# fugue-project/fugue

Measured on AMD Instinct MI355X. Metric: rows_per_sec_transform_fuguesql_groupby_join, higher is better.
Workload: dtype int64+fp64; 1 GPU; model=fuguesql[transform+groupby(sum,count)+join+filter], global_rows=125000000, rows_per_gpu=125000000, n_groups=1000000, dim_rows=1000000, parallelism=dp1, out_rows=1000000

## Files before the change

fugue_amd/hip/csrc/bindings.cpp:

```cpp
#include <torch/extension.h>

#include <c10/hip/HIPStream.h>
#include <hip/hip_runtime.h>

#include <cstdlib>
#include <cstdio>
#include <cstring>
#include <limits>
#include <vector>

#include "relational.h"

namespace {

hipStream_t current_stream() {
  return (hipStream_t)c10::hip::getCurrentHIPStream().stream();
}

void check_gpu(const at::Tensor& t, const char* name) {
  TORCH_CHECK(t.is_cuda(), name, " must be on the GPU");
  TORCH_CHECK(t.is_contiguous(), name, " must be contiguous");
}

const bool* opt_valid_ptr(const c10::optional<at::Tensor>& v) {
// ... 621 lines not shown
  }
  TORCH_CHECK((bin_group_base.slice(0, 1) - bin_group_base.slice(0, 0, nbins))
                      .max()
                      .item<int64_t>() <= 65536,
              "a bin wider than 65536 ids does not fit 16-bit ids");
  auto stream = current_stream();
  auto counts = at::empty({ntiles, nbins}, pos.options());
  launch_scatter_bin_count(pos.data_ptr<int32_t>(), n, (int)tile,
                           bin_offsets.data_ptr<int64_t>(), (int)nbins,
                           counts.data_ptr<int32_t>(), stream);
  auto row_incl = counts.cumsum(1, at::kLong);
  auto start = row_incl - counts;
  auto tile_delta = (bin_offsets.slice(0, 0, nbins).unsqueeze(0) +
                     (counts.cumsum(0, at::kLong) - counts) - start)
                        .to(at::kInt)
                        .contiguous();
  auto tile_start = at::cat({start, row_incl.slice(1, nbins - 1, nbins)}, 1)
                        .to(at::kShort)
                        .contiguous();
  launch_scatter_tile_prep_compact(
      pos.data_ptr<int32_t>(), n, (int)tile, bin_offsets.data_ptr<int64_t>(),
      bin_group_base.data_ptr<int64_t>(), (int)nbins,
      tile_delta.data_ptr<int32_t>(), gid.data_ptr<int32_t>(),
      (uint16_t*)rank.data_ptr<int16_t>(), (uint16_t*)rel.data_ptr<int16_t>(),
      keep_gid ? gid_new.data_ptr<int32_t>() : nullptr, stream);
  std::vector<at::Tensor> res = {rank, rel, tile_start, tile_delta};
  if (keep_gid) res.push_back(gid_new);
  return res;
}

at::Tensor scatter_tile_compact(at::Tensor vals, at::Tensor rank,
                                at::Tensor tile_start, at::Tensor tile_delta,
                                int64_t tile, int64_t threads,
                                c10::optional<at::Tensor> out_opt) {
  if (out_opt.has_value()) {
    check_gpu(*out_opt, "out");
    TORCH_CHECK(out_opt->scalar_type() == at::kDouble &&
                    out_opt->is_contiguous() &&
                    out_opt->numel() == rank.numel(),
                "out must be contiguous fp64 [n]");
  }
  auto out = out_opt.has_value() ? *out_opt
                                 : at::empty({rank.numel()}, vals.options());
  scatter_tile_compact_into(vals, rank, tile_start, tile_delta, tile, threads,
                            out);
  return out;
}

at::Tensor gb_dense_aggregate_compact(at::Tensor rel, at::Tensor pvals,
                                      at::Tensor bin_offsets,
                                      at::Tensor bin_group_base,
                                      at::Tensor bin_chunk_base,
                                      int64_t total_chunks, int64_t n_groups,
                                      int64_t chunk, int64_t slots) {
  TORCH_CHECK(n_groups >= 0 && n_groups < (int64_t(1) << 31),
              "n_groups must fit int32");
  auto out_sum = at::zeros({n_groups}, pvals.options());
  dense_aggregate_compact_into(rel, pvals, bin_offsets, bin_group_base,
                               bin_chunk_base, total_chunks, chunk, slots,
                               out_sum);
  return out_sum;
}

at::Tensor gb_replay_compact(at::Tensor vals, at::Tensor rel, at::Tensor rank,
                             at::Tensor tile_start, at::Tensor tile_delta,
                             at::Tensor bin_offsets,
                             at::Tensor bin_group_base,
                             at::Tensor bin_chunk_base, int64_t total_chunks,
                             int64_t n_groups, int64_t chunk, int64_t slots,
                             int64_t tile, int64_t threads) {
  check_gpu(vals, "vals");
  int64_t n = rel.numel();
  TORCH_CHECK(vals.scalar_type() == at::kDouble && vals.numel() == n,
              "vals must be fp64 [1, n]");
  TORCH_CHECK(n_groups >= 0 && n_groups < (int64_t(1) << 31),
              "n_groups must fit int32");
  TORCH_CHECK(rank.numel() == n, "rank must be int16 [n]");
  auto pvals = at::empty({n}, vals.options());
  scatter_tile_compact_into(vals.view({n}), rank, tile_start, tile_delta, tile,
                            threads, pvals);
  auto out_sum = at::zeros({n_groups}, vals.options());
  if (rel.scalar_type() == at::kInt) {
    dense_aggregate_binned_into(rel, pvals, bin_offsets, bin_group_base,
                                bin_chunk_base, total_chunks, chunk, slots,
                                out_sum);
  } else {
    dense_aggregate_compact_into(rel, pvals, bin_offsets, bin_group_base,
                                 bin_chunk_base, total_chunks, chunk, slots,
                                 out_sum);
  }
  return out_sum;
}

std::vector<at::Tensor> join_build(at::Tensor keys, int64_t tsize) {
  check_gpu(keys, "keys");
  TORCH_CHECK((tsize & (tsize - 1)) == 0, "tsize must be a power of 2");
  int64_t n = keys.numel();
  auto heads = at::full({tsize}, -1, keys.options().dtype(at::kInt));
  auto next = at::empty({std::max<int64_t>(n, 1)},
                        keys.options().dtype(at::kInt));
  auto dup = at::zeros({1}, keys.options().dtype(at::kInt));
  if (n > 0) {
    launch_join_build(keys.data_ptr<int64_t>(), n, heads.data_ptr<int32_t>(),
                      next.data_ptr<int32_t>(), tsize,
                      dup.data_ptr<int32_t>(), current_stream());
  }
  return {heads, next, dup};
}


// ... 16 lines not shown
  auto out_bi = at::empty({np}, pkeys.options());
  auto cursor = at::zeros({1}, pkeys.options());
  auto out_mask = at::empty({want_mask && mode == 1 ? np : 0},
                            pkeys.options().dtype(at::kBool));
  if (np > 0) {
    launch_join_emit_unique(
        pkeys.data_ptr<int64_t>(), np, bkeys.data_ptr<int64_t>(),
        opt_i64_ptr(ph2), opt_i64_ptr(bh2), heads.data_ptr<int32_t>(),
        next.data_ptr<int32_t>(), tsize, (int)mode,
        out_pi.numel() > 0 ? out_pi.data_ptr<int64_t>() : nullptr,
        out_bi.data_ptr<int64_t>(), cursor.data_ptr<int64_t>(),
        out_mask.numel() > 0 ? out_mask.data_ptr<bool>() : nullptr,
        mask_neg ? 1 : 0, current_stream());
  }
  return {out_pi, out_bi, cursor, out_mask};
}

namespace {
void jsel_operand(const py::handle& spec, int s, int64_t np, int64_t nb,
                  JoinSelPred* p) {
  auto t = py::cast<py::tuple>(spec);
  TORCH_CHECK(t.size() == 2, "operand is (kind, value)");
  int kind = py::cast<int>(t[0]);
  p->kind[s] = kind;
  if (kind == JSEL_IMM) {
    if (py::isinstance<py::float_>(t[1])) {
      double d = py::cast<double>(t[1]);
      std::memcpy(&p->imm[s], &d, 8);
      p->is_f64[s] = 1;
    } else {
      TORCH_CHECK(py::isinstance<py::int_>(t[1]) &&
                      !py::isinstance<py::bool_>(t[1]),
                  "immediate must be an int or a float");
      p->imm[s] = (unsigned long long)py::cast<int64_t>(t[1]);
      p->is_f64[s] = 0;
    }
    return;
  }
  TORCH_CHECK(kind == JSEL_PROBE || kind == JSEL_BUILD, "operand kind");
  auto col = py::cast<at::Tensor>(t[1]);
  check_gpu(col, "predicate column");
  TORCH_CHECK(col.scalar_type() == at::kLong ||
                  col.scalar_type() == at::kDouble,
              "predicate columns are int64 or float64");
  TORCH_CHECK(col.numel() == (kind == JSEL_PROBE ? np : nb),
              "predicate column length does not match its side");
  p->ptr[s] = reinterpret_cast<unsigned long long>(col.data_ptr());
  p->is_f64[s] = col.scalar_type() == at::kDouble ? 1 : 0;
}
}

std::vector<at::Tensor> join_unique_select(
    at::Tensor pkeys, at::Tensor bkeys, at::Tensor heads, at::Tensor next,
    py::object pred, std::vector<std::pair<int64_t, at::Tensor>> out_specs) {
  check_gpu(pkeys, "probe_keys");
  check_gpu(bkeys, "build_keys");
  check_gpu(heads, "heads");
  check_gpu(next, "next");
  TORCH_CHECK(pkeys.scalar_type() == at::kLong &&
                  bkeys.scalar_type() == at::kLong,
              "join keys must be int64");
  TORCH_CHECK(heads.scalar_type() == at::kInt &&
                  next.scalar_type() == at::kInt,
              "heads/next must be int32");
  TORCH_CHECK(out_specs.size() >= 1 && out_specs.size() <= COMPACT_MAX_COLS,
              "1..", COMPACT_MAX_COLS, " output columns");
  int64_t np = pkeys.numel(), nb = bkeys.numel();
  int64_t tsize = heads.numel();
  TORCH_CHECK(tsize > 0 && (tsize & (tsize - 1)) == 0,
              "heads length must be a power of 2");
  TORCH_CHECK(next.numel() >= nb, "next is shorter than the build side");
  TORCH_CHECK(nb <= std::numeric_limits<int32_t>::max(),
              "build side too long for int32 chain links");
  bool empty = np == 0 || nb == 0;
  JoinSelPred p;
  std::memset(&p, 0, sizeof(p));
  p.op = -1;
  if (!pred.is_none()) {
    auto t = py::cast<py::tuple>(pred);
    TORCH_CHECK(t.size() == 3, "pred is (op, lhs, rhs)");
    p.op = py::cast<int>(t[0]);
    TORCH_CHECK(p.op >= 0 && p.op <= 5, "comparison op code 0..5");
    jsel_operand(t[1], 0, np, nb, &p);
    jsel_operand(t[2], 1, np, nb, &p);
    p.use_int = (!p.is_f64[0] && !p.is_f64[1]) ? 1 : 0;
  }
  JoinSelCols c;
  std::memset(&c, 0, sizeof(c));
  c.ncols = (int)out_specs.size();
  std::vector<at::Tensor> outs;
  for (size_t i = 0; i < out_specs.size(); ++i) {
    int64_t side = out_specs[i].first;
    const at::Tensor& col = out_specs[i].second;
    TORCH_CHECK(side == JSEL_PROBE || side == JSEL_BUILD, "column side");
    check_gpu(col, "output column");
    TORCH_CHECK(col.element_size() == 8, "8-byte columns only");
    TORCH_CHECK(col.numel() == (side == JSEL_PROBE ? np : nb),
                "output column length does not match its side");
    auto out = at::empty({empty ? 0 : np}, col.options());
    c.side[i] = (int)side;
    c.src[i] = reinterpret_cast<unsigned long long>(col.data_ptr());
    c.dst[i] = reinterpret_cast<unsigned long long>(out.data_ptr());
    outs.push_back(out);
  }
  auto cursor = at::zeros({1}, pkeys.options());
  if (!empty) {
    launch_join_unique_select(
        pkeys.data_ptr<int64_t>(), np, bkeys.data_ptr<int64_t>(),
        heads.data_ptr<int32_t>(), next.data_ptr<int32_t>(), tsize, &p, &c,
        cursor.data_ptr<int64_t>(), current_stream());
  }
  outs.push_back(cursor);
  return outs;
}

at::Tensor join_count(at::Tensor pkeys, at::Tensor bkeys,
                      c10::optional<at::Tensor> ph2,
                      c10::optional<at::Tensor> bh2, at::Tensor heads,
                      at::Tensor next, int64_t tsize) {
  check_gpu(pkeys, "pkeys");
  int64_t np = pkeys.numel();
  auto counts = at::zeros({np}, pkeys.options().dtype(at::kInt));
  if (np > 0) {
    launch_join_count(pkeys.data_ptr<int64_t>(), np,
                      bkeys.data_ptr<int64_t>(), opt_i64_ptr(ph2),
                      opt_i64_ptr(bh2), heads.data_ptr<int32_t>(),
                      next.data_ptr<int32_t>(), tsize,
                      counts.data_ptr<int32_t>(), current_stream());
  }
  return counts;
}

std::vector<at::Tensor> join_pairs(at::Tensor pkeys, at::Tensor bkeys,
                                   c10::optional<at::Tensor> ph2,
                                   c10::optional<at::Tensor> bh2,
                                   at::Tensor heads, at::Tensor next,
                                   int64_t tsize, int64_t mode) {
  check_gpu(pkeys, "pkeys");
  int64_t np = pkeys.numel();
  auto stream = current_stream();
  auto total_t = at::zeros({1}, pkeys.options());
  if (np > 0) {
    launch_join_total(pkeys.data_ptr<int64_t>(), np,
                      bkeys.data_ptr<int64_t>(), opt_i64_ptr(ph2),
                      opt_i64_ptr(bh2), heads.data_ptr<int32_t>(),
                      next.data_ptr<int32_t>(), tsize, (int)mode,
                      total_t.data_ptr<int64_t>(), stream);
  }
  int64_t out_n = total_t.cpu().item<int64_t>();
  auto out_p = at::empty({out_n}, pkeys.options());
  auto out_b = at::empty({out_n}, pkeys.options());
  if (np > 0 && out_n > 0) {
    auto cursor = at::zeros({1}, pkeys.options());
    launch_join_emit_chunked(
        pkeys.data_ptr<int64_t>(), np, bkeys.data_ptr<int64_t>(),
        opt_i64_ptr(ph2), opt_i64_ptr(bh2), heads.data_ptr<int32_t>(),
        next.data_ptr<int32_t>(), tsize, cursor.data_ptr<int64_t>(),
        out_p.data_ptr<int64_t>(), out_b.data_ptr<int64_t>(), (int)mode,
        stream);
  }
  return {out_p, out_b};
}

// ... 672 lines not shown
        py::arg("force_simple"), py::arg("record_chunk") = 0);
  m.def("dense_assign_max", []() { return (int64_t)DENSE_ASSIGN_MAX; },
        "largest per-partition distinct count the dense layout accepts");
  m.def("gb_dense_count", &gb_dense_count,
        "dense replay preparation: offsets + distinct keys per partition",
        py::arg("pkeys"), py::arg("num_parts"));
  m.def("gb_dense_assign", &gb_dense_assign,
        "dense replay preparation: group ids, output keys and counts",
        py::arg("pkeys"), py::arg("offsets"), py::arg("group_base"),
        py::arg("n_groups"));
  m.def("scatter_tile_prepare", &scatter_tile_prepare,
        "tile-coalesced scatter preparation (rank, dst) of a permutation");
  m.def("scatter_tile", &scatter_tile, "tile-coalesced value scatter");
  m.def("gb_dense_aggregate", &gb_dense_aggregate,
        "sum per dense group id (LDS table per chunk)", py::arg("gid"),
        py::arg("pvals"), py::arg("offsets"), py::arg("group_base"),
        py::arg("n_groups"), py::arg("chunk"), py::arg("slots"));
  m.def("gb_replay_dense", &gb_replay_dense,
        "replayed step: value scatter + dense aggregate", py::arg("vals"),
        py::arg("gid"), py::arg("offsets"), py::arg("group_base"),
        py::arg("n_groups"), py::arg("chunk"), py::arg("slots"),
        py::arg("tile") = 0, py::arg("rank") = py::none(),
        py::arg("dst") = py::none(), py::arg("pos") = py::none());
  m.def("scatter_tile_prepare_binned", &scatter_tile_prepare_binned,
        "tile scatter preparation into the binned layout: rank, dst, gid",
        py::arg("pos"), py::arg("gid"), py::arg("bin_offsets"),
        py::arg("tile"));
  m.def("gb_dense_aggregate_binned", &gb_dense_aggregate_binned,
        "sum per dense group id over the binned layout", py::arg("gid"),
        py::arg("pvals"), py::arg("bin_offsets"), py::arg("bin_group_base"),
        py::arg("bin_chunk_base"), py::arg("total_chunks"),
        py::arg("n_groups"), py::arg("chunk"), py::arg("slots"));
  m.def("gb_replay_binned", &gb_replay_binned,
        "replayed step over the binned layout: scatter + aggregate",
        py::arg("vals"), py::arg("gid"), py::arg("rank"), py::arg("dst"),
        py::arg("bin_offsets"), py::arg("bin_group_base"),
        py::arg("bin_chunk_base"), py::arg("total_chunks"),
        py::arg("n_groups"), py::arg("chunk"), py::arg("slots"),
        py::arg("tile"));
  m.def("scatter_tile_prepare_compact", &scatter_tile_prepare_compact,
        "compact binned preparation: rank, rel, tile_start, tile_delta",
        py::arg("pos"), py::arg("gid"), py::arg("bin_offsets"),
        py::arg("bin_group_base"), py::arg("tile"),
        py::arg("keep_gid") = false);
  m.def("scatter_tile_compact", &scatter_tile_compact,
        "tile-coalesced value scatter over the compact binned layout",
        py::arg("vals"), py::arg("rank"), py::arg("tile_start"),
        py::arg("tile_delta"), py::arg("tile"), py::arg("threads") = 0,
        py::arg("out") = py::none());
  m.def("gb_dense_aggregate_compact", &gb_dense_aggregate_compact,
        "sum per group over the binned layout, 16-bit ids", py::arg("rel"),
        py::arg("pvals"), py::arg("bin_offsets"), py::arg("bin_group_base"),
        py::arg("bin_chunk_base"), py::arg("total_chunks"),
        py::arg("n_groups"), py::arg("chunk"), py::arg("slots"));
  m.def("gb_replay_compact", &gb_replay_compact,
        "replayed step over the compact binned layout: scatter + aggregate",
        py::arg("vals"), py::arg("rel"), py::arg("rank"),
        py::arg("tile_start"), py::arg("tile_delta"), py::arg("bin_offsets"),
        py::arg("bin_group_base"), py::arg("bin_chunk_base"),
        py::arg("total_chunks"), py::arg("n_groups"), py::arg("chunk"),
        py::arg("slots"), py::arg("tile"), py::arg("threads") = 0);
  m.attr("COMPACT_CHUNK") = (int64_t)COMPACT_CHUNK;
  m.attr("COMPACT_MAX_COLS") = (int64_t)COMPACT_MAX_COLS;
  m.def("join_build",&join_build, "build chained hash table");
  m.def("join_unique_select", &join_unique_select,
        "unique inner join + residual comparison + projection, one pass",
        py::arg("probe_keys"), py::arg("build_keys"), py::arg("heads"),
        py::arg("next"), py::arg("pred"), py::arg("out_specs"));
  m.def("join_emit_unique", &join_emit_unique,
        "single-pass join emit for unique build keys");
  m.def("hash_string_column", &hash_string_column,
        "combine a string column into the running row hash");
  m.def("hash_seed", &hash_seed, "seed a row-hash buffer");
  m.def("gb_mark_reps", &gb_mark_reps,
        "representative rows + h2 verification for hashed group-by");
  m.def("expr_value", &expr_value,
        "fused value-expression interpreter");
  m.def("expr_filter", &expr_filter,
        "fused filter-predicate interpreter");
  m.def("gather_columns", &gather_columns,
        "fused multi-column row gather");
  m.def("gb_key_stats", &gb_key_stats,
        "fused key min/max + sampled distinct estimate");
  m.def("pack_columns", &pack_columns, "pack key columns into int64");
  m.def("unpack_column", &unpack_column, "unpack one key column");
  m.def("seg_rank_chunk", &seg_rank_chunk,
        "sorted positions per block of the segmented rank kernels");
  m.def("seg_rank", &seg_rank,
        "segmented row_number/rank/dense_rank in original row order");
  m.def("seg_take", &seg_take,
        "deterministic first-n-per-segment index vector");
  m.def("seg_shift", &seg_shift,
        "segment-bounded shift (LAG/LEAD) in original row order");
  m.def("seg_scan", &seg_scan,
        "segmented running sum/min/max + non-null count");
  m.def("seg_total", &seg_total,
        "whole-partition sum/min/max/first/last + non-null count");
  m.def("seg_frame_tile", &seg_frame_tile,
        "sorted positions per block of the frame kernel");
  m.def("seg_frame_max_reach", &seg_frame_max_reach,
        "largest frame reach the frame kernel takes");
  m.def("seg_frame", &seg_frame,
        "moving-frame sum/min/max/first/last + non-null count");
  m.def("gb_compact", &gb_compact,
        "deterministic group-table compaction");
  m.def("compact_columns_cap", &compact_columns_cap,
        "mask compaction, capacity outputs + cursor");
  m.def("join_open_unique", &join_open_unique,
        "open-addressed unique int join (build+probe)");
  m.def("topk_select", &topk_select, "own top-k (k<=16) select");
  m.def("eq2_mask", &eq2_mask, "128-bit string equality mask");
  m.def("cmp_imm", &cmp_imm, "single col-vs-literal comparison mask");
  m.def("cmp_col", &cmp_col, "single col-vs-col comparison mask");
  m.def("compact_columns", &compact_columns,
        "fused masked compaction of 8-byte columns");
  m.def("join_count", &join_count, "count matches per probe row");
  m.def("join_emit", &join_emit, "emit join pairs");
  m.def("reduce_columns", &reduce_columns,
        "global column reductions (MFMA-reduced sums)");
  m.def("join_pairs", &join_pairs,
        "total + chunked-reservation join pair emission");
// ... 3 lines not shown
```

fugue_amd/hip/csrc/groupby_replay.hip:

```cpp
#include <hip/hip_runtime.h>

#include "device_common.h"
#include "relational.h"


__global__ __launch_bounds__(BLOCK) void scatter_by_pos_kernel(
    const double* __restrict__ vals, const int32_t* __restrict__ pos,
    int64_t n, double* __restrict__ out_vals) {
  int64_t stride = (int64_t)gridDim.x * blockDim.x;
  for (int64_t i = (int64_t)blockIdx.x * blockDim.x + threadIdx.x; i < n;
       i += stride) {
    out_vals[pos[i]] = vals[i];
  }
}

extern "C" {
void launch_scatter_by_pos(const double* vals, const int32_t* pos, int64_t n,
                           double* out_vals, hipStream_t stream) {
  hipLaunchKernelGGL(scatter_by_pos_kernel, dim3(grid_for(n, 2)), dim3(BLOCK),
                     0, stream, vals, pos, n, out_vals);
}
}


// ... 438 lines not shown
    if (end > bin_end) end = bin_end;
    if (start < 0) start = 0;
    if (end > n) end = n;
    const int base = (int)bin_group_base[b];
    __syncthreads();
    int64_t i = start + threadIdx.x;
    const int64_t stride = (int64_t)blockDim.x;
    for (; i + 3 * stride < end; i += 4 * stride) {
      int g[4];
      double v[4];
#pragma unroll
      for (int u = 0; u < 4; ++u) g[u] = gid[i + u * stride];
#pragma unroll
      for (int u = 0; u < 4; ++u) v[u] = part_vals[i + u * stride];
#pragma unroll
      for (int u = 0; u < 4; ++u) {
        unsigned rel = (unsigned)(g[u] - base);
        if (rel < (unsigned)SLOTS) {
          atomicAdd(&lsum[rel], v[u]);
        } else if ((uint64_t)g[u] < (uint64_t)n_groups) {
          atomicAdd(&out_sum[g[u]], v[u]);
        }
      }
    }
    for (; i < end; i += stride) {
      int g = gid[i];
      double v = part_vals[i];
      unsigned rel = (unsigned)(g - base);
      if (rel < (unsigned)SLOTS) {
        atomicAdd(&lsum[rel], v);
      } else if ((uint64_t)g < (uint64_t)n_groups) {
        atomicAdd(&out_sum[g], v);
      }
    }
    __syncthreads();
    for (int s = threadIdx.x; s < SLOTS; s += blockDim.x) {
      double v = lsum[s];
      if (v != 0.0 && (int64_t)base + s < n_groups)
        atomicAdd(&out_sum[(int64_t)base + s], v);
    }
    __syncthreads();
  }
}

template <int SLOTS>
__global__ __launch_bounds__(BLOCK) void gb_dense_aggregate_compact_kernel(
    const uint16_t* __restrict__ rel, const double* __restrict__ part_vals,
    int64_t n, const int64_t* __restrict__ bin_offsets,
    const int64_t* __restrict__ bin_group_base,
    const int64_t* __restrict__ bin_chunk_base, int nbins,
    int64_t total_chunks, int64_t n_groups, double* __restrict__ out_sum,
    int64_t chunk) {
  __shared__ double lsum[SLOTS];
  for (int64_t vc = blockIdx.x; vc < total_chunks; vc += gridDim.x) {
    for (int i = threadIdx.x; i < SLOTS; i += blockDim.x) lsum[i] = 0.0;
    const int b = bin_of(bin_chunk_base, nbins, vc);
    int64_t start = bin_offsets[b] + (vc - bin_chunk_base[b]) * chunk;
    int64_t end = start + chunk;
    const int64_t bin_end = bin_offsets[b + 1];
    if (end > bin_end) end = bin_end;
    if (start < 0) start = 0;
    if (end > n) end = n;
    const int64_t base = bin_group_base[b];
    __syncthreads();
    auto add = [&](unsigned g, double v) {
      if (g < (unsigned)SLOTS) {
        atomicAdd(&lsum[g], v);
      } else if ((uint64_t)(base + g) < (uint64_t)n_groups) {
        atomicAdd(&out_sum[base + g], v);
      }
    };
    int64_t a0 = (start + 3) & ~(int64_t)3;
    if (a0 > end) a0 = end;
    const int64_t a1 = a0 + ((end - a0) & ~(int64_t)3);
    {
      int64_t h = start + threadIdx.x;
      if (h < a0) add(rel[h], part_vals[h]);
      int64_t t = a1 + threadIdx.x;
      if (t < end) add(rel[t], part_vals[t]);
    }
    const int64_t stride = (int64_t)blockDim.x * 4;
    int64_t i = a0 + (int64_t)threadIdx.x * 4;
    for (; i + stride < a1; i += 2 * stride) {
      uint2 g0 = *(const uint2*)(rel + i);
      uint2 g1 = *(const uint2*)(rel + i + stride);
      double2 v0 = *(const double2*)(part_vals + i);
      double2 v1 = *(const double2*)(part_vals + i + 2);
      double2 v2 = *(const double2*)(part_vals + i + stride);
      double2 v3 = *(const double2*)(part_vals + i + stride + 2);
      add(g0.x & 0xffffu, v0.x);
      add(g0.x >> 16, v0.y);
      add(g0.y & 0xffffu, v1.x);
      add(g0.y >> 16, v1.y);
      add(g1.x & 0xffffu, v2.x);
      add(g1.x >> 16, v2.y);
      add(g1.y & 0xffffu, v3.x);
      add(g1.y >> 16, v3.y);
    }
    if (i < a1) {
      uint2 g0 = *(const uint2*)(rel + i);
      double2 v0 = *(const double2*)(part_vals + i);
      double2 v1 = *(const double2*)(part_vals + i + 2);
      add(g0.x & 0xffffu, v0.x);
      add(g0.x >> 16, v0.y);
      add(g0.y & 0xffffu, v1.x);
      add(g0.y >> 16, v1.y);
    }
    __syncthreads();
    for (int s = threadIdx.x; s < SLOTS; s += blockDim.x) {
      double v = lsum[s];
      if (v != 0.0 && (uint64_t)(base + s) < (uint64_t)n_groups)
        atomicAdd(&out_sum[base + s], v);
    }
    __syncthreads();
  }
}

extern "C" {

void launch_gb_dense_count(const int64_t* pkeys, const int64_t* offsets,
                           int num_parts, int64_t* distinct,
                           hipStream_t stream) {
  hipLaunchKernelGGL(gb_dense_count_kernel, dim3(num_parts), dim3(BLOCK), 0,
                     stream, pkeys, offsets, num_parts, distinct);
}

void launch_gb_dense_assign(const int64_t* pkeys, const int64_t* offsets,
                            const int64_t* group_base, int num_parts,
                            int32_t* gid, int64_t* out_keys,
                            int64_t* out_count, hipStream_t stream) {
  hipLaunchKernelGGL(gb_dense_assign_kernel, dim3(num_parts), dim3(BLOCK), 0,
                     stream, pkeys, offsets, group_base, num_parts, gid,
                     out_keys, out_count);
}

void launch_scatter_tile_prep(const int32_t* pos, int64_t n, int tile,
                              uint16_t* rank, int32_t* dst,
                              hipStream_t stream) {
  hipLaunchKernelGGL(scatter_tile_prep_kernel, dim3(chunk_grid(n, tile)),
                     dim3(BLOCK), (size_t)tile * sizeof(unsigned long long),
                     stream, pos, n, tile, rank, dst);
}

void launch_scatter_tile(const double* vals, const uint16_t* rank,
                         const int32_t* dst, int64_t n, int tile,
                         double* out, hipStream_t stream) {
  hipLaunchKernelGGL(scatter_tile_kernel, dim3(chunk_grid(n, tile)),
                     dim3(BLOCK), (size_t)tile * sizeof(double), stream, vals,
                     rank, dst, n, tile, out);
}

void launch_gb_dense_aggregate(const int32_t* gid, const double* part_vals,
                               int64_t n, const int64_t* offsets,
                               const int64_t* group_base, int num_parts,
                               int64_t n_groups, double* out_sum,
                               int64_t chunk, int slots,
                               hipStream_t stream) {
  if (chunk <= 0) chunk = BLOCK * 128;
  dim3 g(chunk_grid(n, chunk)), b(BLOCK);
  switch (slots) {
    case 2048:
      hipLaunchKernelGGL((gb_dense_aggregate_kernel<2048>), g, b, 0, stream,
                         gid, part_vals, n, offsets, group_base, num_parts,
                         n_groups, out_sum, chunk);
      break;
    case 8192:
      hipLaunchKernelGGL((gb_dense_aggregate_kernel<8192>), g, b, 0, stream,
// ... 49 lines not shown
                         n_groups, out_sum, chunk);
      break;
    default:
      hipLaunchKernelGGL((gb_dense_aggregate_binned_kernel<8192>), g, b, 0,
                         stream, gid, part_vals, n, bin_offsets,
                         bin_group_base, bin_chunk_base, nbins, total_chunks,
                         n_groups, out_sum, chunk);
  }
}


void launch_scatter_tile_prep_compact(
    const int32_t* pos, int64_t n, int tile, const int64_t* bin_offsets,
    const int64_t* bin_group_base, int nbins, const int32_t* tile_delta,
    const int32_t* gid_old, uint16_t* rank, uint16_t* rel, int32_t* gid_new,
    hipStream_t stream) {
  hipLaunchKernelGGL(scatter_tile_prep_compact_kernel,
                     dim3(chunk_grid(n, tile)), dim3(BLOCK),
                     (size_t)tile * sizeof(unsigned long long), stream, pos, n,
                     tile, bin_offsets, bin_group_base, nbins, tile_delta,
                     gid_old, rank, rel, gid_new);
}

}

namespace {
template <int NT>
hipError_t scatter_tile_compact_launch(
    const double* vals, const uint16_t* rank, const uint16_t* tile_start,
    const int32_t* tile_delta, int nbins, int64_t n, int tile, double* out,
    hipStream_t stream) {
  size_t lds = (size_t)tile * sizeof(double) + (size_t)nbins * 4 +
               (((size_t)nbins + 1) * 2 + 7) / 8 * 8;
  if (lds > 65536) {
    static bool opted[64] = {};
    int dev = 0;
    hipError_t e = hipGetDevice(&dev);
    if (e != hipSuccess) return e;
    if (dev < 0 || dev >= 64 || !opted[dev]) {
      e = hipFuncSetAttribute(
          reinterpret_cast<const void*>(&scatter_tile_compact_kernel<NT>),
          hipFuncAttributeMaxDynamicSharedMemorySize,
          8192 * 8 + SCATTER_COMPACT_MAX_BINS * 4 +
              (SCATTER_COMPACT_MAX_BINS + 8) * 2);
      if (e != hipSuccess) return e;
      if (dev >= 0 && dev < 64) opted[dev] = true;
    }
  }
  hipLaunchKernelGGL((scatter_tile_compact_kernel<NT>),
                     dim3(chunk_grid(n, tile)), dim3(NT), lds, stream, vals,
                     rank, tile_start, tile_delta, nbins, n, tile, out);
  return hipGetLastError();
}
}

extern "C" {

int launch_scatter_tile_compact(const double* vals, const uint16_t* rank,
                                const uint16_t* tile_start,
                                const int32_t* tile_delta, int nbins,
                                int64_t n, int tile, double* out, int threads,
                                hipStream_t stream) {
  switch (threads) {
    case 512:
      return (int)scatter_tile_compact_launch<512>(
          vals, rank, tile_start, tile_delta, nbins, n, tile, out, stream);
    default:
      return (int)scatter_tile_compact_launch<1024>(
          vals, rank, tile_start, tile_delta, nbins, n, tile, out, stream);
  }
}

void launch_gb_dense_aggregate_compact(
    const uint16_t* rel, const double* part_vals, int64_t n,
    const int64_t* bin_offsets, const int64_t* bin_group_base,
    const int64_t* bin_chunk_base, int nbins, int64_t total_chunks,
    int64_t n_groups, double* out_sum, int64_t chunk, int slots,
    hipStream_t stream) {
  dim3 g(chunk_grid(total_chunks, 1)), b(BLOCK);
  switch (slots) {
    case 2048:
      hipLaunchKernelGGL((gb_dense_aggregate_compact_kernel<2048>), g, b, 0,
                         stream, rel, part_vals, n, bin_offsets,
                         bin_group_base, bin_chunk_base, nbins, total_chunks,
                         n_groups, out_sum, chunk);
      break;
    case 4096:
      hipLaunchKernelGGL((gb_dense_aggregate_compact_kernel<4096>), g, b, 0,
                         stream, rel, part_vals, n, bin_offsets,
                         bin_group_base, bin_chunk_base, nbins, total_chunks,
                         n_groups, out_sum, chunk);
      break;
    default:
      hipLaunchKernelGGL((gb_dense_aggregate_compact_kernel<8192>), g, b, 0,
                         stream, rel, part_vals, n, bin_offsets,
                         bin_group_base, bin_chunk_base, nbins, total_chunks,
                         n_groups, out_sum, chunk);
  }
}

}
```

fugue_amd/hip/csrc/join.hip:

```cpp
#include <hip/hip_runtime.h>

#include "device_common.h"
#include "relational.h"


__global__ __launch_bounds__(BLOCK) void join_build_kernel(
    const int64_t* __restrict__ keys, int64_t n,
    int32_t* __restrict__ heads,
    int32_t* __restrict__ next,
    int64_t tsize) {
  int64_t stride = (int64_t)gridDim.x * blockDim.x;
  for (int64_t i = (int64_t)blockIdx.x * blockDim.x + threadIdx.x; i < n;
       i += stride) {
    uint64_t h = mix64((uint64_t)keys[i]);
    int64_t slot = (int64_t)(h & (uint64_t)(tsize - 1));
    int32_t old = atomicExch(&heads[slot], (int32_t)i);
    next[i] = old;
  }
}

__global__ __launch_bounds__(BLOCK) void join_dup_check_kernel(
    const int64_t* __restrict__ keys, int64_t n,
    const int32_t* __restrict__ heads, const int32_t* __restrict__ next,
    int64_t tsize, int32_t* __restrict__ dup) {
// ... 269 lines not shown
            break;
          }
        }
        cur = next[cur];
      }
      if (!any && (mode == 1 || mode == 3)) {
        out_p[pos] = i;
        out_b[pos] = -1;
        ++pos;
      }
    }
  }
}

__global__ __launch_bounds__(BLOCK) void join_mark_build_kernel(
    const int64_t* __restrict__ pkeys, int64_t np,
    const int64_t* __restrict__ bkeys,
    const int64_t* __restrict__ ph2, const int64_t* __restrict__ bh2,
    const int32_t* __restrict__ heads, const int32_t* __restrict__ next,
    int64_t tsize, bool* __restrict__ bmatched) {
  int64_t stride = (int64_t)gridDim.x * blockDim.x;
  for (int64_t i = (int64_t)blockIdx.x * blockDim.x + threadIdx.x; i < np;
       i += stride) {
    int64_t key = pkeys[i];
    uint64_t h = mix64((uint64_t)key);
    int32_t cur = heads[(int64_t)(h & (uint64_t)(tsize - 1))];
    while (cur >= 0) {
      if (bkeys[cur] == key && (ph2 == nullptr || bh2[cur] == ph2[i]))
        bmatched[cur] = true;
      cur = next[cur];
    }
  }
}


__device__ __forceinline__ long long jsel_operand(const JoinSelPred& p, int s,
                                                  int64_t i, int32_t m) {
  if (p.kind[s] == JSEL_IMM) return (long long)p.imm[s];
  const long long* col = reinterpret_cast<const long long*>(p.ptr[s]);
  return p.kind[s] == JSEL_BUILD ? col[m] : col[i];
}

__device__ __forceinline__ bool jsel_pred(const JoinSelPred& p, int64_t i,
                                          int32_t m) {
  if (p.op < 0) return true;
  long long a = jsel_operand(p, 0, i, m);
  long long b = jsel_operand(p, 1, i, m);
  if (p.use_int) return cmp_apply<long long>(a, b, p.op);
  double x = p.is_f64[0] ? __longlong_as_double(a) : (double)a;
  double y = p.is_f64[1] ? __longlong_as_double(b) : (double)b;
  return cmp_apply<double>(x, y, p.op);
}

__global__ __launch_bounds__(BLOCK) void join_unique_select_kernel(
    const int64_t* __restrict__ pkeys, int64_t np,
    const int64_t* __restrict__ bkeys, const int32_t* __restrict__ heads,
    const int32_t* __restrict__ next, int64_t tsize, JoinSelPred pred,
    JoinSelCols cols, int64_t* __restrict__ cursor) {
  __shared__ int32_t smatch[COMPACT_CHUNK];
  __shared__ int lcount;
  __shared__ long long lbase;
  uint64_t tmask = (uint64_t)(tsize - 1);
  for (int64_t start = (int64_t)blockIdx.x * COMPACT_CHUNK; start < np;
       start += (int64_t)gridDim.x * COMPACT_CHUNK) {
    int64_t end = start + COMPACT_CHUNK;
    if (end > np) end = np;
    if (threadIdx.x == 0) lcount = 0;
    __syncthreads();
    int local = 0;
    for (int g = 0; g < COMPACT_CHUNK / BLOCK; g += 4) {
      int64_t idx[4], key[4];
      int32_t cur[4], match[4];
#pragma unroll
      for (int j = 0; j < 4; ++j) {
        idx[j] = start + (int64_t)(g + j) * BLOCK + threadIdx.x;
        match[j] = -1;
        if (idx[j] < end) {
          key[j] = pkeys[idx[j]];
          cur[j] = heads[(int64_t)(mix64((uint64_t)key[j]) & tmask)];
        } else {
          cur[j] = -1;
        }
      }
      bool any = true;
      while (any) {
        any = false;
#pragma unroll
        for (int j = 0; j < 4; ++j) {
          if (cur[j] >= 0) {
            int32_t c = cur[j];
            if (bkeys[c] == key[j]) {
              match[j] = c;
              cur[j] = -1;
            } else {
              cur[j] = next[c];
              if (cur[j] >= 0) any = true;
            }
          }
        }
      }
#pragma unroll
      for (int j = 0; j < 4; ++j) {
        if (match[j] >= 0 && !jsel_pred(pred, idx[j], match[j])) match[j] = -1;
        smatch[(g + j) * BLOCK + threadIdx.x] = match[j];
        if (match[j] >= 0) ++local;
      }
    }
    atomicAdd(&lcount, local);
    __syncthreads();
    if (threadIdx.x == 0) {
      lbase = lcount > 0
                  ? (long long)atomicAdd((unsigned long long*)cursor,
                                         (unsigned long long)lcount)
                  : 0;
      lcount = 0;
    }
    __syncthreads();
    for (int r = 0; r < COMPACT_CHUNK / BLOCK; ++r) {
      int32_t m = smatch[r * BLOCK + threadIdx.x];
      if (m < 0) continue;
      int64_t i = start + (int64_t)r * BLOCK + threadIdx.x;
      int64_t pos = (int64_t)lbase + atomicAdd(&lcount, 1);
#pragma unroll
      for (int c = 0; c < COMPACT_MAX_COLS; ++c) {
        if (c < cols.ncols) {
          const uint64_t* src = reinterpret_cast<const uint64_t*>(cols.src[c]);
          reinterpret_cast<uint64_t*>(cols.dst[c])[pos] =
              cols.side[c] == JSEL_BUILD ? src[m] : src[i];
        }
      }
    }
    __syncthreads();
  }
}

extern "C" {

void launch_join_unique_select(const int64_t* pkeys, int64_t np,
                               const int64_t* bkeys, const int32_t* heads,
                               const int32_t* next, int64_t tsize,
                               const JoinSelPred* pred,
                               const JoinSelCols* cols, int64_t* cursor,
                               hipStream_t stream) {
  hipLaunchKernelGGL(join_unique_select_kernel,
                     dim3(chunk_grid(np, COMPACT_CHUNK)), dim3(BLOCK), 0,
                     stream, pkeys, np, bkeys, heads, next, tsize, *pred,
                     *cols, cursor);
}

void launch_join_build(const int64_t* keys, int64_t n, int32_t* heads,
                       int32_t* next, int64_t tsize, int32_t* dup,
                       hipStream_t stream) {
  hipLaunchKernelGGL(join_build_kernel, dim3(grid_for(n)), dim3(BLOCK), 0,
                     stream, keys, n, heads, next, tsize);
  if (dup != nullptr) {
    hipLaunchKernelGGL(join_dup_check_kernel, dim3(grid_for(n)), dim3(BLOCK),
                       0, stream, keys, n, heads, next, tsize, dup);
  }
}

void launch_join_emit_unique(const int64_t* pkeys, int64_t np,
                             const int64_t* bkeys, const int64_t* ph2,
                             const int64_t* bh2, const int32_t* heads,
                             const int32_t* next, int64_t tsize, int mode,
                             int64_t* out_pi, int64_t* out_bi,
                             int64_t* cursor, bool* out_mask, int mask_neg,
                             hipStream_t stream) {
  if (mode == 1) {
    hipLaunchKernelGGL(join_left_unique_kernel, dim3(grid_for(np, 4)),
                       dim3(BLOCK), 0, stream, pkeys, np, bkeys, ph2, bh2,
                       heads, next, tsize, out_pi, out_bi, out_mask,
                       mask_neg);
  } else {
    hipLaunchKernelGGL(join_emit_unique_kernel, dim3(grid_for(np)),
                       dim3(BLOCK), 0, stream, pkeys, np, bkeys, ph2, bh2,
                       heads, next, tsize, mode, out_pi, out_bi, cursor);
  }
}

void launch_join_count(const int64_t* pkeys, int64_t np, const int64_t* bkeys,
                       const int64_t* ph2, const int64_t* bh2,
                       const int32_t* heads, const int32_t* next,
                       int64_t tsize, int32_t* counts, hipStream_t stream) {
  hipLaunchKernelGGL(join_count_kernel, dim3(grid_for(np)), dim3(BLOCK), 0,
                     stream, pkeys, np, bkeys, ph2, bh2, heads, next, tsize,
                     counts);
}

void launch_join_total(const int64_t* pkeys, int64_t np,
                       const int64_t* bkeys, const int64_t* ph2,
                       const int64_t* bh2, const int32_t* heads,
                       const int32_t* next, int64_t tsize, int mode,
                       int64_t* total, hipStream_t stream) {
  hipLaunchKernelGGL(join_total_kernel, dim3(grid_for(np, 4)), dim3(BLOCK), 0,
                     stream, pkeys, np, bkeys, ph2, bh2, heads, next, tsize,
                     mode, total);
}

void launch_join_emit_chunked(const int64_t* pkeys, int64_t np,
                              const int64_t* bkeys, const int64_t* ph2,
// ... 149 lines not shown
```

fugue_amd/hip/csrc/relational.h:

```cpp
#pragma once

#include <hip/hip_runtime_api.h>

#include <cstdint>

#define BLOCK 256

#define GB_EMPTY 0x8000000000000000LL
#define GB_LDS_MAX_AGGS 4
#define PART_MAX 4096
#define DENSE_ASSIGN_MAX 2048
#define BIN_MAX 4096
#define SCATTER_COMPACT_MAX_BINS 512

#define PACK_MAX_COLS 8
#define GBC_MAX_AGGS 6
#define GBC_CHUNK (BLOCK * 32)

#define GATHER_MAX_COLS 16

#define COMPACT_CHUNK (BLOCK * 16)
#define COMPACT_MAX_COLS 8

enum { JSEL_PROBE = 0, JSEL_BUILD = 1, JSEL_IMM = 2 };
// ... 153 lines not shown
    hipStream_t stream);
int launch_scatter_tile_compact(const double* vals, const uint16_t* rank,
                                const uint16_t* tile_start,
                                const int32_t* tile_delta, int nbins,
                                int64_t n, int tile, double* out, int threads,
                                hipStream_t stream);
void launch_gb_dense_aggregate_compact(
    const uint16_t* rel, const double* part_vals, int64_t n,
    const int64_t* bin_offsets, const int64_t* bin_group_base,
    const int64_t* bin_chunk_base, int nbins, int64_t total_chunks,
    int64_t n_groups, double* out_sum, int64_t chunk, int slots,
    hipStream_t stream);

void launch_join_build(const int64_t* keys, int64_t n, int32_t* heads,
                       int32_t* next, int64_t tsize, int32_t* dup,
                       hipStream_t stream);
void launch_join_emit_unique(const int64_t* pkeys, int64_t np,
                             const int64_t* bkeys, const int64_t* ph2,
                             const int64_t* bh2, const int32_t* heads,
                             const int32_t* next, int64_t tsize, int mode,
                             int64_t* out_pi, int64_t* out_bi,
                             int64_t* cursor, bool* out_mask, int mask_neg,
                             hipStream_t stream);
void launch_join_count(const int64_t* pkeys, int64_t np, const int64_t* bkeys,
                       const int64_t* ph2, const int64_t* bh2,
                       const int32_t* heads, const int32_t* next,
                       int64_t tsize, int32_t* counts, hipStream_t stream);
void launch_join_total(const int64_t* pkeys, int64_t np,
                       const int64_t* bkeys, const int64_t* ph2,
                       const int64_t* bh2, const int32_t* heads,
                       const int32_t* next, int64_t tsize, int mode,
                       int64_t* total, hipStream_t stream);
void launch_join_emit_chunked(const int64_t* pkeys, int64_t np,
                              const int64_t* bkeys, const int64_t* ph2,
                              const int64_t* bh2, const int32_t* heads,
                              const int32_t* next, int64_t tsize,
                              int64_t* cursor, int64_t* out_p,
                              int64_t* out_b, int mode, hipStream_t stream);
void launch_join_emit(const int64_t* pkeys, int64_t np, const int64_t* bkeys,
                      const int64_t* ph2, const int64_t* bh2,
                      const int32_t* heads, const int32_t* next, int64_t tsize,
                      const int64_t* offsets, int64_t* out_p, int64_t* out_b,
                      int mode, hipStream_t stream);
void launch_join_mark_build(const int64_t* pkeys, int64_t np,
                            const int64_t* bkeys, const int64_t* ph2,
                            const int64_t* bh2, const int32_t* heads,
                            const int32_t* next, int64_t tsize, bool* bmatched,
                            hipStream_t stream);
void launch_join_unique_select(const int64_t* pkeys, int64_t np,
                               const int64_t* bkeys, const int32_t* heads,
                               const int32_t* next, int64_t tsize,
                               const JoinSelPred* pred,
                               const JoinSelCols* cols, int64_t* cursor,
                               hipStream_t stream);
void launch_joinoa_build(const int64_t* bkeys, int64_t nb, int64_t* table,
                         int64_t tsize, int64_t* flags, hipStream_t stream);
void launch_joinoa_probe(const int64_t* pkeys, int64_t np,
                         const int64_t* table, int64_t tsize,
                         int64_t* out_pi, int64_t* out_bi, bool* out_mask,
                         int mask_neg, hipStream_t stream);

void launch_gather_cols(const uint64_t* src_ptrs, const uint64_t* dst_ptrs,
                        int ncols, int elem_size, const int64_t* idx,
                        int64_t n, hipStream_t stream);
void launch_expr_filter(const ExprProg* prog, int64_t n, bool* out,
                        hipStream_t stream);
void launch_expr_value(const ExprProg* prog, int64_t n, int out_int,
                       void* out_v, bool* out_valid, hipStream_t stream);
void launch_compact8(const bool* mask, int64_t n, int64_t* cursor,
                     const uint64_t** srcs, uint64_t** dsts, int ncols,
                     hipStream_t stream);
void launch_cmp_imm(const void* a, const bool* valid, int dtype,
                    int64_t imm_i, double imm_d, int use_int, int op,
                    int64_t n, bool* out, hipStream_t stream);
void launch_cmp_col(const void* a, const bool* va, const void* b,
                    const bool* vb, int dtype, int op, int64_t n, bool* out,
                    hipStream_t stream);
void launch_eq2_mask(const int64_t* h1, const int64_t* h2, const int64_t* l1,
                     const int64_t* l2, const bool* valid, int neg,
                     int64_t n, bool* out, hipStream_t stream);
void launch_topk(const void* vals, int dtype, int largest, int64_t n, int k,
                 void* cand_v, int64_t* cand_i, void* out_v, int64_t* out_i,
                 hipStream_t stream);

void launch_gb_compact(const int64_t* tkeys, const int64_t* gcount,
                       const double** agg_src, double** agg_dst, int n_aggs,
                       int64_t tsize, int64_t* bcounts, int64_t* bases,
                       int64_t* out_keys, int64_t* out_count,
                       const int64_t* extra_src, int64_t* extra_dst,
                       hipStream_t stream);
void launch_seg_rank(const int64_t* perm, const int64_t* pkeys,
                     const int64_t* const* col_data,
                     const uint8_t* const* col_valid, const int* col_is_float,
                     int ncols, int64_t n, int kind, int64_t* work,
                     int64_t* out, hipStream_t stream);
void launch_seg_take(const int64_t* perm, const int64_t* pkeys, int64_t n,
                     int64_t n_take, int64_t* work, int64_t* bcounts,
                     int64_t* bases, int64_t* out, hipStream_t stream);
void launch_seg_shift(const int64_t* perm, const int64_t* pkeys,
                      const int64_t* vals, const uint8_t* valid, int64_t n,
                      int64_t d, int64_t* out, uint8_t* out_valid,
                      hipStream_t stream);
void launch_seg_scan(const int64_t* perm, const int64_t* pkeys,
                     const int64_t* vals, const uint8_t* valid, int64_t n,
                     int op, int is_float, int64_t* work, int64_t* out_acc,
                     int64_t* out_cnt, hipStream_t stream);
void launch_seg_total(const int64_t* perm, const int64_t* pkeys,
// ... 10 lines not shown
```

Before: 84.01 billion rows/s.

## Rebalance dense aggregate with contiguous chunk ranges and adaptive join block size

```diff
diff --git a/fugue_amd/hip/csrc/bindings.cpp b/fugue_amd/hip/csrc/bindings.cpp
--- a/fugue_amd/hip/csrc/bindings.cpp
+++ b/fugue_amd/hip/csrc/bindings.cpp
@@ -697,10 +697,19 @@
                                       at::Tensor bin_group_base,
                                       at::Tensor bin_chunk_base,
                                       int64_t total_chunks, int64_t n_groups,
-                                      int64_t chunk, int64_t slots) {
+                                      int64_t chunk, int64_t slots,
+                                      c10::optional<at::Tensor> out_opt) {
   TORCH_CHECK(n_groups >= 0 && n_groups < (int64_t(1) << 31),
               "n_groups must fit int32");
-  auto out_sum = at::zeros({n_groups}, pvals.options());
+  if (out_opt.has_value()) {
+    check_gpu(*out_opt, "out");
+    TORCH_CHECK(out_opt->scalar_type() == at::kDouble &&
+                    out_opt->is_contiguous() && out_opt->dim() == 1 &&
+                    out_opt->numel() >= n_groups,
+                "out must be contiguous fp64 of at least n_groups");
+  }
+  auto out_sum = out_opt.has_value() ? out_opt->narrow(0, 0, n_groups)
+                                     : at::zeros({n_groups}, pvals.options());
   dense_aggregate_compact_into(rel, pvals, bin_offsets, bin_group_base,
                                bin_chunk_base, total_chunks, chunk, slots,
                                out_sum);
@@ -823,7 +832,12 @@
 
 std::vector<at::Tensor> join_unique_select(
     at::Tensor pkeys, at::Tensor bkeys, at::Tensor heads, at::Tensor next,
-    py::object pred, std::vector<std::pair<int64_t, at::Tensor>> out_specs) {
+    py::object pred, std::vector<std::pair<int64_t, at::Tensor>> out_specs,
+    int64_t block_rows) {
+  TORCH_CHECK(block_rows == 0 || block_rows == 1024 || block_rows == 2048 ||
+                  block_rows == COMPACT_CHUNK,
+              "block_rows is 0 (by probe length), 1024, 2048 or ",
+              COMPACT_CHUNK);
   check_gpu(pkeys, "probe_keys");
   check_gpu(bkeys, "build_keys");
   check_gpu(heads, "heads");
@@ -879,7 +893,7 @@
     launch_join_unique_select(
         pkeys.data_ptr<int64_t>(), np, bkeys.data_ptr<int64_t>(),
         heads.data_ptr<int32_t>(), next.data_ptr<int32_t>(), tsize, &p, &c,
-        cursor.data_ptr<int64_t>(), current_stream());
+        cursor.data_ptr<int64_t>(), (int)block_rows, current_stream());
   }
   outs.push_back(cursor);
   return outs;
@@ -1658,7 +1672,8 @@
         "sum per group over the binned layout, 16-bit ids", py::arg("rel"),
         py::arg("pvals"), py::arg("bin_offsets"), py::arg("bin_group_base"),
         py::arg("bin_chunk_base"), py::arg("total_chunks"),
-        py::arg("n_groups"), py::arg("chunk"), py::arg("slots"));
+        py::arg("n_groups"), py::arg("chunk"), py::arg("slots"),
+        py::arg("out") = py::none());
   m.def("gb_replay_compact", &gb_replay_compact,
         "replayed step over the compact binned layout: scatter + aggregate",
         py::arg("vals"), py::arg("rel"), py::arg("rank"),
@@ -1672,7 +1687,8 @@
   m.def("join_unique_select", &join_unique_select,
         "unique inner join + residual comparison + projection, one pass",
         py::arg("probe_keys"), py::arg("build_keys"), py::arg("heads"),
-        py::arg("next"), py::arg("pred"), py::arg("out_specs"));
+        py::arg("next"), py::arg("pred"), py::arg("out_specs"),
+        py::arg("block_rows") = 0);
   m.def("join_emit_unique", &join_emit_unique,
         "single-pass join emit for unique build keys");
   m.def("hash_string_column", &hash_string_column,
diff --git a/fugue_amd/hip/csrc/groupby_replay.hip b/fugue_amd/hip/csrc/groupby_replay.hip
--- a/fugue_amd/hip/csrc/groupby_replay.hip
+++ b/fugue_amd/hip/csrc/groupby_replay.hip
@@ -514,17 +514,28 @@
     int64_t total_chunks, int64_t n_groups, double* __restrict__ out_sum,
     int64_t chunk) {
   __shared__ double lsum[SLOTS];
-  for (int64_t vc = blockIdx.x; vc < total_chunks; vc += gridDim.x) {
-    for (int i = threadIdx.x; i < SLOTS; i += blockDim.x) lsum[i] = 0.0;
+  const int tid = threadIdx.x;
+  const int64_t q = total_chunks / gridDim.x, rem = total_chunks % gridDim.x;
+  const int64_t bx = blockIdx.x;
+  int64_t vc = bx * q + (bx < rem ? bx : rem);
+  const int64_t vc1 = vc + q + (bx < rem ? 1 : 0);
+  if (vc >= vc1) return;
+  for (int i = tid; i < SLOTS; i += BLOCK) lsum[i] = 0.0;
+  __syncthreads();
+  while (vc < vc1) {
     const int b = bin_of(bin_chunk_base, nbins, vc);
-    int64_t start = bin_offsets[b] + (vc - bin_chunk_base[b]) * chunk;
-    int64_t end = start + chunk;
+    const int64_t cb = bin_chunk_base[b];
+    int64_t ve = bin_chunk_base[b + 1];
+    if (ve > vc1) ve = vc1;
+    if (ve <= vc) ve = vc + 1;
+    const int64_t base = bin_group_base[b];
+    int64_t start = bin_offsets[b] + (vc - cb) * chunk;
+    int64_t end = bin_offsets[b] + (ve - cb) * chunk;
     const int64_t bin_end = bin_offsets[b + 1];
     if (end > bin_end) end = bin_end;
     if (start < 0) start = 0;
     if (end > n) end = n;
-    const int64_t base = bin_group_base[b];
-    __syncthreads();
+    if (start > end) start = end;
     auto add = [&](unsigned g, double v) {
       if (g < (unsigned)SLOTS) {
         atomicAdd(&lsum[g], v);
@@ -534,47 +545,52 @@
     };
     int64_t a0 = (start + 3) & ~(int64_t)3;
     if (a0 > end) a0 = end;
-    const int64_t a1 = a0 + ((end - a0) & ~(int64_t)3);
-    {
-      int64_t h = start + threadIdx.x;
+    const int64_t ng = (end - a0) >> 2;
+    const int64_t a1 = a0 + (ng << 2);
+    if (tid < 4) {
+      int64_t h = start + tid;
       if (h < a0) add(rel[h], part_vals[h]);
-      int64_t t = a1 + threadIdx.x;
+      int64_t t = a1 + tid;
       if (t < end) add(rel[t], part_vals[t]);
     }
-    const int64_t stride = (int64_t)blockDim.x * 4;
-    int64_t i = a0 + (int64_t)threadIdx.x * 4;
-    for (; i + stride < a1; i += 2 * stride) {
-      uint2 g0 = *(const uint2*)(rel + i);
-      uint2 g1 = *(const uint2*)(rel + i + stride);
-      double2 v0 = *(const double2*)(part_vals + i);
-      double2 v1 = *(const double2*)(part_vals + i + 2);
-      double2 v2 = *(const double2*)(part_vals + i + stride);
-      double2 v3 = *(const double2*)(part_vals + i + stride + 2);
-      add(g0.x & 0xffffu, v0.x);
-      add(g0.x >> 16, v0.y);
-      add(g0.y & 0xffffu, v1.x);
-      add(g0.y >> 16, v1.y);
-      add(g1.x & 0xffffu, v2.x);
-      add(g1.x >> 16, v2.y);
-      add(g1.y & 0xffffu, v3.x);
-      add(g1.y >> 16, v3.y);
-    }
-    if (i < a1) {
-      uint2 g0 = *(const uint2*)(rel + i);
-      double2 v0 = *(const double2*)(part_vals + i);
-      double2 v1 = *(const double2*)(part_vals + i + 2);
-      add(g0.x & 0xffffu, v0.x);
-      add(g0.x >> 16, v0.y);
-      add(g0.y & 0xffffu, v1.x);
-      add(g0.y >> 16, v1.y);
-    }
-    __syncthreads();
-    for (int s = threadIdx.x; s < SLOTS; s += blockDim.x) {
+    if (ng > 0) {
+      const uint16_t* rp = rel + a0;
+      const double* vp = part_vals + a0;
+      uint2 ga, gb;
+      double2 va0, va1, vb0, vb1;
+      auto load = [&](uint2& g, double2& v0, double2& v1, int64_t j) {
+        if (j >= ng) j = ng - 1;
+        g = *(const uint2*)(rp + 4 * j);
+        v0 = *(const double2*)(vp + 4 * j);
+        v1 = *(const double2*)(vp + 4 * j + 2);
+      };
+      auto consume = [&](uint2 g, double2 v0, double2 v1, int64_t j) {
+        if (j < ng) {
+          add(g.x & 0xffffu, v0.x);
+          add(g.x >> 16, v0.y);
+          add(g.y & 0xffffu, v1.x);
+          add(g.y >> 16, v1.y);
+        }
+      };
+      load(ga, va0, va1, tid);
+      for (int64_t j = tid; j < ng; j += 2 * BLOCK) {
+        load(gb, vb0, vb1, j + BLOCK);
+        consume(ga, va0, va1, j);
+        load(ga, va0, va1, j + 2 * BLOCK);
+        consume(gb, vb0, vb1, j + BLOCK);
+      }
+    }
+    vc = ve;
+    __syncthreads();
+    for (int s = tid; s < SLOTS; s += BLOCK) {
       double v = lsum[s];
-      if (v != 0.0 && (uint64_t)(base + s) < (uint64_t)n_groups)
-        atomicAdd(&out_sum[base + s], v);
-    }
-    __syncthreads();
+      if (v != 0.0) {
+        if ((uint64_t)(base + s) < (uint64_t)n_groups)
+          atomicAdd(&out_sum[base + s], v);
+        lsum[s] = 0.0;
+      }
+    }
+    if (vc < vc1) __syncthreads();
   }
 }
 
@@ -730,6 +746,41 @@
                      rank, tile_start, tile_delta, nbins, n, tile, out);
   return hipGetLastError();
 }
+
+template <int SLOTS>
+void dense_aggregate_compact_launch(
+    const uint16_t* rel, const double* part_vals, int64_t n,
+    const int64_t* bin_offsets, const int64_t* bin_group_base,
+    const int64_t* bin_chunk_base, int nbins, int64_t total_chunks,
+    int64_t n_groups, double* out_sum, int64_t chunk, hipStream_t stream) {
+  static int resident[64] = {};
+  int dev = 0;
+  if (hipGetDevice(&dev) != hipSuccess) dev = -1;
+  int grid = dev >= 0 && dev < 64 ? resident[dev] : 0;
+  if (grid == 0) {
+    int cus = 0, per_cu = 0;
+    if (dev < 0 ||
+        hipDeviceGetAttribute(&cus, hipDeviceAttributeMultiprocessorCount,
+                              dev) != hipSuccess ||
+        cus < 1)
+      cus = 256;
+    if (hipOccupancyMaxActiveBlocksPerMultiprocessor(
+            &per_cu,
+            reinterpret_cast<const void*>(
+                &gb_dense_aggregate_compact_kernel<SLOTS>),
+            BLOCK, 0) != hipSuccess ||
+        per_cu < 1)
+      per_cu = 1;
+    grid = cus * per_cu;
+    if (grid > MAX_GRID) grid = MAX_GRID;
+    if (dev >= 0 && dev < 64) resident[dev] = grid;
+  }
+  if (total_chunks < grid) grid = (int)total_chunks;
+  hipLaunchKernelGGL((gb_dense_aggregate_compact_kernel<SLOTS>), dim3(grid),
+                     dim3(BLOCK), 0, stream, rel, part_vals, n, bin_offsets,
+                     bin_group_base, bin_chunk_base, nbins, total_chunks,
+                     n_groups, out_sum, chunk);
+}
 }
 
 extern "C" {
@@ -755,26 +806,22 @@
     const int64_t* bin_chunk_base, int nbins, int64_t total_chunks,
     int64_t n_groups, double* out_sum, int64_t chunk, int slots,
     hipStream_t stream) {
-  dim3 g(chunk_grid(total_chunks, 1)), b(BLOCK);
   switch (slots) {
     case 2048:
-      hipLaunchKernelGGL((gb_dense_aggregate_compact_kernel<2048>), g, b, 0,
-                         stream, rel, part_vals, n, bin_offsets,
-                         bin_group_base, bin_chunk_base, nbins, total_chunks,
-                         n_groups, out_sum, chunk);
+      dense_aggregate_compact_launch<2048>(
+          rel, part_vals, n, bin_offsets, bin_group_base, bin_chunk_base,
+          nbins, total_chunks, n_groups, out_sum, chunk, stream);
       break;
     case 4096:
-      hipLaunchKernelGGL((gb_dense_aggregate_compact_kernel<4096>), g, b, 0,
-                         stream, rel, part_vals, n, bin_offsets,
-                         bin_group_base, bin_chunk_base, nbins, total_chunks,
-                         n_groups, out_sum, chunk);
+      dense_aggregate_compact_launch<4096>(
+          rel, part_vals, n, bin_offsets, bin_group_base, bin_chunk_base,
+          nbins, total_chunks, n_groups, out_sum, chunk, stream);
       break;
     default:
-      hipLaunchKernelGGL((gb_dense_aggregate_compact_kernel<8192>), g, b, 0,
-                         stream, rel, part_vals, n, bin_offsets,
-                         bin_group_base, bin_chunk_base, nbins, total_chunks,
-                         n_groups, out_sum, chunk);
-  }
-}
-
-}
+      dense_aggregate_compact_launch<8192>(
+          rel, part_vals, n, bin_offsets, bin_group_base, bin_chunk_base,
+          nbins, total_chunks, n_groups, out_sum, chunk, stream);
+  }
+}
+
+}
diff --git a/fugue_amd/hip/csrc/join.hip b/fugue_amd/hip/csrc/join.hip
--- a/fugue_amd/hip/csrc/join.hip
+++ b/fugue_amd/hip/csrc/join.hip
@@ -345,23 +345,25 @@
   return cmp_apply<double>(x, y, p.op);
 }
 
+template <int ROWS>
 __global__ __launch_bounds__(BLOCK) void join_unique_select_kernel(
     const int64_t* __restrict__ pkeys, int64_t np,
     const int64_t* __restrict__ bkeys, const int32_t* __restrict__ heads,
     const int32_t* __restrict__ next, int64_t tsize, JoinSelPred pred,
     JoinSelCols cols, int64_t* __restrict__ cursor) {
-  __shared__ int32_t smatch[COMPACT_CHUNK];
+  static_assert(ROWS % (4 * BLOCK) == 0, "whole rounds of four rows");
+  __shared__ int32_t smatch[ROWS];
   __shared__ int lcount;
   __shared__ long long lbase;
   uint64_t tmask = (uint64_t)(tsize - 1);
-  for (int64_t start = (int64_t)blockIdx.x * COMPACT_CHUNK; start < np;
-       start += (int64_t)gridDim.x * COMPACT_CHUNK) {
-    int64_t end = start + COMPACT_CHUNK;
+  for (int64_t start = (int64_t)blockIdx.x * ROWS; start < np;
+       start += (int64_t)gridDim.x * ROWS) {
+    int64_t end = start + ROWS;
     if (end > np) end = np;
     if (threadIdx.x == 0) lcount = 0;
     __syncthreads();
     int local = 0;
-    for (int g = 0; g < COMPACT_CHUNK / BLOCK; g += 4) {
+    for (int g = 0; g < ROWS / BLOCK; g += 4) {
       int64_t idx[4], key[4];
       int32_t cur[4], match[4];
 #pragma unroll
@@ -409,7 +411,7 @@
       lcount = 0;
     }
     __syncthreads();
-    for (int r = 0; r < COMPACT_CHUNK / BLOCK; ++r) {
+    for (int r = 0; r < ROWS / BLOCK; ++r) {
       int32_t m = smatch[r * BLOCK + threadIdx.x];
       if (m < 0) continue;
       int64_t i = start + (int64_t)r * BLOCK + threadIdx.x;
@@ -427,6 +429,23 @@
   }
 }
 
+namespace {
+int device_cus() {
+  static int cus[64] = {};
+  int dev = 0;
+  if (hipGetDevice(&dev) != hipSuccess || dev < 0 || dev >= 64) return 256;
+  if (cus[dev] == 0) {
+    int c = 0;
+    if (hipDeviceGetAttribute(&c, hipDeviceAttributeMultiprocessorCount,
+                              dev) != hipSuccess ||
+        c < 1)
+      c = 256;
+    cus[dev] = c;
+  }
+  return cus[dev];
+}
+}
+
 extern "C" {
 
 void launch_join_unique_select(const int64_t* pkeys, int64_t np,
@@ -434,11 +453,25 @@
                                const int32_t* next, int64_t tsize,
                                const JoinSelPred* pred,
                                const JoinSelCols* cols, int64_t* cursor,
-                               hipStream_t stream) {
-  hipLaunchKernelGGL(join_unique_select_kernel,
-                     dim3(chunk_grid(np, COMPACT_CHUNK)), dim3(BLOCK), 0,
-                     stream, pkeys, np, bkeys, heads, next, tsize, *pred,
-                     *cols, cursor);
+                               int block_rows, hipStream_t stream) {
+  if (block_rows <= 0) {
+    const int64_t want = (int64_t)4 * device_cus();
+    block_rows = COMPACT_CHUNK;
+    while (block_rows > 1024 && np / block_rows < want) block_rows /= 2;
+  }
+#define JSEL_RUN(ROWS)                                                     \
+  hipLaunchKernelGGL(join_unique_select_kernel<ROWS>,                      \
+                     dim3(chunk_grid(np, ROWS)), dim3(BLOCK), 0, stream,   \
+                     pkeys, np, bkeys, heads, next, tsize, *pred, *cols,   \
+                     cursor)
+  if (block_rows >= COMPACT_CHUNK) {
+    JSEL_RUN(COMPACT_CHUNK);
+  } else if (block_rows >= 2048) {
+    JSEL_RUN(2048);
+  } else {
+    JSEL_RUN(1024);
+  }
+#undef JSEL_RUN
 }
 
 void launch_join_build(const int64_t* keys, int64_t n, int32_t* heads,
diff --git a/fugue_amd/hip/csrc/relational.h b/fugue_amd/hip/csrc/relational.h
--- a/fugue_amd/hip/csrc/relational.h
+++ b/fugue_amd/hip/csrc/relational.h
@@ -229,7 +229,7 @@
                                const int32_t* next, int64_t tsize,
                                const JoinSelPred* pred,
                                const JoinSelCols* cols, int64_t* cursor,
-                               hipStream_t stream);
+                               int block_rows, hipStream_t stream);
 void launch_joinoa_build(const int64_t* bkeys, int64_t nb, int64_t* table,
                          int64_t tsize, int64_t* flags, hipStream_t stream);
 void launch_joinoa_probe(const int64_t* pkeys, int64_t np,
```

New measurement: 86.35 billion rows/s (median of 6 runs). 1.03x the previous value.
